# BDMstudio/audio-cut

Measured on AMD Instinct MI355X. Metric: audio-seconds processed/sec (separate+detect) per GPU; cut-point index parity, higher is better.
Workload: dtype f32

## Files before the change

### audio_cut_amd/_native.py

```python
from __future__ import annotations

import ctypes as C
import threading
import os
from pathlib import Path
from typing import Optional, Sequence, Tuple

import numpy as np
import torch

_LIB_NAME = "libaudiocut_hip.so"
_lib: Optional[C.CDLL] = None


class NativeError(RuntimeError):
    pass


def library_path() -> Path:
    return Path(__file__).resolve().parent / os.environ.get("AUDIOCUT_HIP_LIBNAME", _LIB_NAME)


def load() -> C.CDLL:
    global _lib
    if _lib is not None:
        return _lib
    path = library_path()
    if not path.exists():
        raise NativeError(f"{path} is missing: build it with `make -C audio_cut_amd/csrc` "
                          f"(there is no CPU fallback for the HIP path)")
    lib = C.CDLL(str(path))
    _declare(lib)
    if lib.ac_abi_version() != 6:
        raise NativeError("libaudiocut_hip.so ABI version mismatch")
    if lib.ac_stereo_abi_version() != 1:
        raise NativeError("libaudiocut_hip.so stereo ABI version mismatch")
    if lib.ac_onset_abi_version() != 1:
        raise NativeError("libaudiocut_hip.so onset ABI version mismatch")
    if lib.ac_beat_abi_version() != 1:
        raise NativeError("libaudiocut_hip.so beat ABI version mismatch")
    if lib.ac_hybrid_abi_version() != 1:
        raise NativeError("libaudiocut_hip.so hybrid ABI version mismatch")
    if lib.ac_export_abi_version() != 1:
        raise NativeError("libaudiocut_hip.so export ABI version mismatch")
    if lib.ac_asr_abi_version() != 1:
        raise NativeError("libaudiocut_hip.so asr ABI version mismatch")
    if lib.ac_profile_abi_version() != 1:
        raise NativeError("libaudiocut_hip.so profile ABI version mismatch")
    _lib = lib
    return lib


_P = C.c_void_p
_I64 = C.c_int64
_I = C.c_int

SIGNATURES = {
    "ac_abi_version": (C.c_int, []),
    "ac_last_error": (C.c_char_p, []),
    "ac_ctx_create": (C.c_int, [_I, C.POINTER(_P)]),
    "ac_ctx_destroy": (C.c_int, [_P]),
    "ac_frame_rms": (C.c_int, [_P, _P, _I64, _I, _I, _I, _P, _I64, _P]),
    "ac_frame_rms_multi": (C.c_int, [_P, _P, _I64, _I, _P, _P, _P, _P, _P]),
    "ac_stft2048_features": (C.c_int, [_P, _P, _I64, _I, _P, _P, _P, _P, _P, _I64, _P]),
    "ac_onset_strength": (C.c_int, [_P, _P, _I64, _P, _I, _I, _I, _P, _P, _P]),
    "ac_tempogram_parts": (C.c_int, [_I64]),
    "ac_tempogram_reduce": (C.c_int, [_P, _P, _I64, _I, _P, _P, _P, _P, _P]),
    "ac_yin_f0": (C.c_int, [_P, _P, _I64, _I, _I, _I, _I, C.c_double, _P, _P, _I64, _P]),
    "ac_moving_meansq_db_f64": (C.c_int, [_P, _P, _I64, _I, _P, _P]),
    "ac_next_leq_scratch": (C.c_int64, [_I64]),
    "ac_next_leq_scan": (C.c_int, [_P, _P, _I64, C.c_double, _P, _P, _P]),
    "ac_window_argmin_f64": (C.c_int, [_P, _P, _I64, _P, _P, _I, _P, _P, _P]),
    "ac_zero_cross_nearest": (C.c_int, [_P, _P, _I64, _P, _I, _I, _P, _P]),
    "ac_quiet_guard_slow": (C.c_int, [_P, _P, _I64, _P, _I, _I, _I, _P, _P, _P]),
    "ac_pause_cut_points": (C.c_int, [_P, _P, _I64, _P, _P, _I, _I, _I, _P, _P, _P]),
    "ac_mdx_stft": (C.c_int, [_P, _P, _I64, _P, _P, _P, _I, _P, _P, _P]),
    "ac_mdx_istft": (C.c_int, [_P, _P, _I, _P, _P, _P]),
    "ac_mdx_assemble_ola": (C.c_int, [_P, _P, _I64, _P, _P, _P, _P, _P, _P, _I, _P, _P, _P]),
    "ac_mdx_chunk_vocal": (C.c_int, [_P, _P, _P, _P, _P, _I, _P, _P]),
    "ac_sum_squares": (C.c_int, [_P, _P, _I64, _P, _I, _P]),
    "ac_window_sum_squares": (C.c_int, [_P, _P, _I64, _P, _P, _I, _P, _P]),
# ... 35 lines not shown


ONSET_SIGNATURES = {
    "ac_onset_abi_version": (C.c_int, []),
    "ac_bar_energy_silence": (C.c_int, [_P, _P, _I64, _P, _P, _I, C.c_double, _P, _P, _P]),
    "ac_segment_pair_energy": (C.c_int, [_P, _P, _P, _I64, _P, _P, _I, _P, _P]),
}

BEAT_SIGNATURES = {
    "ac_beat_abi_version": (C.c_int, []),
    "ac_stft2048_centroid_bandwidth": (C.c_int, [_P, _P, _I64, _I, C.c_double, _P, _P, _I64, _P]),
    "ac_bar_means3": (C.c_int, [_P, _P, _I64, _P, _P, _I64, _P, _P, _I, _P, _P]),
}

HYBRID_SIGNATURES = {
    "ac_hybrid_abi_version": (C.c_int, []),
    "ac_quiet_gate_meansq": (C.c_int, [_P, _P, _I64, _I64, _P, _I, _P, _I64, _P, _P, _P]),
}

EXPORT_SIGNATURES = {
    "ac_export_abi_version": (C.c_int, []),
    "ac_mdx_assemble_pcm24": (C.c_int, [_P, _P, _I64, _I, _P, _P, _P, _P, _P, _P, _I, _P, _P, _P, _I, _P]),
}

ASR_SIGNATURES = {
    "ac_asr_abi_version": (C.c_int, []),
    "ac_resample_poly_pcm16": (C.c_int, [_P, _P, _I64, _I, _I, _P, _I64, _I64, _P, _I64, _P]),
}

PROFILE_SIGNATURES = {
    "ac_profile_abi_version": (C.c_int, []),
    "ac_abs_peak_coverage": (C.c_int, [_P, _P, _I64, C.c_double, C.c_double, _P, _P, _P, _P]),
}
PROFILE_GRID_SAMPLES = 4 * 256 * 2048


def coverage_from(peak: float, count: int, n: int) -> float:
    if int(n) == 0 or float(peak) <= 1e-9:
        return 0.0
    return max(0.0, min(1.0, int(count) / int(n)))


def _declare(lib: C.CDLL) -> None:
    for name, (res, args) in (*SIGNATURES.items(), *STEREO_SIGNATURES.items(), *ONSET_SIGNATURES.items(), *BEAT_SIGNATURES.items(),
                              *HYBRID_SIGNATURES.items(), *EXPORT_SIGNATURES.items(), *ASR_SIGNATURES.items(), *PROFILE_SIGNATURES.items()):
        fn = getattr(lib, name)
        fn.restype = res
        fn.argtypes = args


def _check(rc: int) -> None:
    if rc != 0:
        msg = load().ac_last_error()
        raise NativeError(f"libaudiocut_hip call failed ({rc}): {msg.decode() if msg else '?'}")


def _ptr(t: Optional[torch.Tensor]) -> Optional[int]:
    if t is None:
        return None
    if not t.is_contiguous():
        raise NativeError("non-contiguous tensor passed to the HIP ABI")
    return t.data_ptr()


def _stream() -> int:
    return torch.cuda.current_stream().cuda_stream


def _packed(name: str, t: Optional[torch.Tensor], n_bytes: Optional[int]) -> None:
    if t is None or n_bytes is None:
        return
    have = t.numel() * t.element_size()
    if have != n_bytes:
        raise NativeError(f"{name}: the packed weights hold {have} bytes, the shape implies {n_bytes} (see separation/conv_pack.py)")


def _conv3x3_packed_bytes(c_in: int, c_out: int, cob: int, stage: int) -> Optional[int]:
    if c_in <= 0 or c_out <= 0 or c_in % 16 or c_out % cob:
# ... 708 lines not shown
    def conv3x3_f16x3_first(self, spec: torch.Tensor, w1: torch.Tensor, b1: torch.Tensor, w_packed: torch.Tensor, bias: torch.Tensor,
                            c_out: int, w_unscale: float, relu: bool = True, spec_amax: Optional[torch.Tensor] = None,
                            amax_gain: float = 1.0, amax_offs: float = 0.0, out_amax: Optional[torch.Tensor] = None) -> torch.Tensor:
        if spec.dtype != torch.float32 or spec.dim() != 4 or not spec.is_contiguous():
            raise NativeError("conv3x3_f16x3_first expects a contiguous float32 NCHW tensor")
        b, c0, h, w = spec.shape
        w1 = w1.reshape(w1.shape[0], -1)
        if w1.shape[1] != c0 or not w1.is_contiguous():
            raise NativeError("conv3x3_f16x3_first: w1 must be [C_in, C0(,1,1)] contiguous")
        _packed("conv3x3_f16x3_first", w_packed, _conv3x3_packed_bytes(w1.shape[0], int(c_out), 48, 8))
        out = torch.empty((b, c_out, h, w), dtype=torch.float32, device=self.device)
        pi, po = self._amax_args(b, spec_amax, out_amax, h, h)
        _check(self.lib.ac_conv3x3_f16x3_first(self._h, _ptr(spec), _ptr(w1), _ptr(b1), _ptr(w_packed), _ptr(bias), _ptr(out), b, c0,
                                               w1.shape[0], c_out, h, w, float(w_unscale), int(relu), pi, float(amax_gain),
                                               float(amax_offs), po, _stream()))
        return out

    def tdf_linear_f16x3(self, x: torch.Tensor, w_packed: torch.Tensor, n_out: int, scale: torch.Tensor, shift: torch.Tensor,
                         w_unscale: float, resid: Optional[torch.Tensor] = None, in_amax: Optional[torch.Tensor] = None,
                         out_amax: Optional[torch.Tensor] = None) -> torch.Tensor:
        if x.dtype != torch.float32 or x.dim() != 4 or not x.is_contiguous():
            raise NativeError("tdf_linear_f16x3 expects a contiguous float32 NCHW tensor")
        b, c, t, k = x.shape
        if c % 16 == 0 and t % 8 == 0:
            _packed("tdf_linear_f16x3", w_packed, _linear_packed_bytes(int(n_out), k, 0))
        out = torch.empty((b, c, t, n_out), dtype=torch.float32, device=self.device)
        if resid is not None and (resid.shape != out.shape or not resid.is_contiguous() or resid.dtype != torch.float32):
            raise NativeError("tdf_linear_f16x3: residual must match the output")
        pi, po = self._amax_args(b, in_amax, out_amax, t, t)
        _check(self.lib.ac_tdf_linear_f16x3(self._h, _ptr(x), _ptr(w_packed), _ptr(scale), _ptr(shift), _ptr(resid), _ptr(out),
                                            b * c * t, n_out, k, t, c, float(w_unscale), pi, po, _stream()))
        return out

    def tdf_small_fused(self, x: torch.Tensor, w1_packed: torch.Tensor, w2_packed: torch.Tensor, hidden: int, scale1: torch.Tensor,
                        shift1: torch.Tensor, scale2: torch.Tensor, shift2: torch.Tensor,
                        out_amax: Optional[torch.Tensor] = None) -> torch.Tensor:
        if x.dtype != torch.float32 or x.dim() != 4 or not x.is_contiguous():
            raise NativeError("tdf_small_fused expects a contiguous float32 NCHW tensor")
        b, c, t, f = x.shape
        hd = int(hidden)
        if f > 0 and f % 32 == 0 and 0 < hd <= 48 and (b * c * t) % 32 == 0:
            _packed("tdf_small_fused (w1)", w1_packed, -(-hd // 16) * (f // 16) * 64 * 4 * 4)
            _packed("tdf_small_fused (w2)", w2_packed, (f // 16) * -(-hd // 4) * 64 * 4)
        out = torch.empty_like(x)
        _, po = self._amax_args(b, None, out_amax, t, t)
        _check(self.lib.ac_tdf_small_fused(self._h, _ptr(x), _ptr(w1_packed), _ptr(w2_packed), _ptr(scale1), _ptr(shift1), _ptr(scale2),
                                           _ptr(shift2), _ptr(out), b * c * t, f, int(hidden), t, c, po, _stream()))
        return out

    def conv1x1_small(self, x: torch.Tensor, weight: torch.Tensor, bias: torch.Tensor, relu: bool) -> torch.Tensor:
        if x.dtype != torch.float32 or x.dim() != 4 or not x.is_contiguous():
            raise NativeError("conv1x1_small expects a contiguous float32 NCHW tensor")
        b, c, h, w = x.shape
        w2 = weight.reshape(weight.shape[0], -1)
        if w2.shape[1] != c or not w2.is_contiguous():
            raise NativeError("conv1x1_small: weight must be [C_out, C_in(,1,1)] contiguous")
        _packed("conv1x1_small (bias)", bias, w2.shape[0] * 4)
        out = torch.empty((b, w2.shape[0], h, w), dtype=torch.float32, device=self.device)
        _check(self.lib.ac_conv1x1_small(self._h, _ptr(x), _ptr(w2), _ptr(bias), _ptr(out), b, c, w2.shape[0], h * w, int(relu), _stream()))
        return out

    def down2x_f16x3(self, x: torch.Tensor, w_packed: torch.Tensor, bias: torch.Tensor, c_out: int, w_unscale: float,
                     in_amax: Optional[torch.Tensor] = None, out_amax: Optional[torch.Tensor] = None) -> torch.Tensor:
        if x.dtype != torch.float32 or x.dim() != 4 or not x.is_contiguous():
            raise NativeError("down2x_f16x3 expects a contiguous float32 NCHW tensor")
        b, c, h, w = x.shape
# ... 69 lines not shown
```

### audio_cut_amd/csrc/ac_gemm.hip

```cpp
#include "ac_common.h"
#include <stdlib.h>
#ifndef GM_RESID_AHEAD
#define GM_RESID_AHEAD 0
#endif
#ifndef AC_PROBES
#define AC_PROBES 0
#endif

typedef __attribute__((ext_vector_type(8))) _Float16 f16x8;
typedef __attribute__((ext_vector_type(4))) float f32x4;

#define GM_BM 128
#define GM_BK 32
#define GM_ASTRIDE 48
#define GM_MT 4
#define GM_A_ITERS ((GM_BM * (GM_BK / 4)) / 256)

__device__ inline unsigned short gm_f16_bits(_Float16 h) { return __builtin_bit_cast(unsigned short, h); }

template <int NT, bool RESID>
__global__ __launch_bounds__(256, 2) void k_tdf_linear_f16x3(const float* __restrict__ x, const f16x8* __restrict__ wpk,
                                                             const float* __restrict__ scale, const float* __restrict__ shift,
                                                             const float* __restrict__ resid, float* __restrict__ y,
                                                             int n_mblk, int N, int K, int T, int C, float w_unscale,
                                                             const float* __restrict__ in_amax, float* __restrict__ out_amax,
                                                             int ord_g, int ord_r) {
    constexpr int BN = 32 * NT;
    constexpr int BFRAGS = 2 * (BN / 16) * 64;
    constexpr int B_ITERS = BFRAGS / 256;
    constexpr int OSTRIDE = 16 * NT + 4;
    constexpr int A_BYTES = 2 * GM_BM * GM_ASTRIDE * 2;
    constexpr int O_BYTES = 4 * 16 * OSTRIDE * 4;
    constexpr int R_BYTES = (RESID && GM_RESID_AHEAD) ? 2 * (16 * (16 * NT) * 4) : 0;
    constexpr int K_ARENA = A_BYTES + 2 * BFRAGS * 16, E_ARENA = O_BYTES + 4 * R_BYTES;
    constexpr int ARENA = K_ARENA > E_ARENA ? K_ARENA : E_ARENA;
    __shared__ __attribute__((aligned(16))) unsigned char s_raw[ARENA];
    unsigned short* s_hi = reinterpret_cast<unsigned short*>(s_raw);
    unsigned short* s_lo = s_hi + GM_BM * GM_ASTRIDE;
    f16x8* s_b0 = reinterpret_cast<f16x8*>(s_raw + A_BYTES);
    f16x8* s_b1 = s_b0 + BFRAGS;
    float* s_out = reinterpret_cast<float*>(s_raw);

    const int tid = threadIdx.x, lane = tid & 63, wave = tid >> 6;
    const int wm = wave >> 1, wn = wave & 1;
    const int n_nblk = N / BN;
    int wi = blockIdx.x;
    if ((gridDim.x & 7) == 0) wi = (blockIdx.x & 7) * (gridDim.x >> 3) + (blockIdx.x >> 3);
    const int per = ord_r * n_nblk;
    const int chunk = wi / per, i_in = wi - chunk * per;
    const int nb_hi = i_in / (ord_g * ord_r), j_in = i_in - nb_hi * (ord_g * ord_r);
    const int nb = nb_hi * ord_g + j_in % ord_g, mb = chunk * ord_r + j_in / ord_g;
    if (mb >= n_mblk) return;
    const int n0 = nb * BN;
    const int n_stage = K / GM_BK;
    const int n_blk = T / 8, n_cg = C / 16;
    const int tb = mb % n_blk, cg = (mb / n_blk) % n_cg, item = mb / (n_blk * n_cg);
    const size_t m_base = ((size_t)item * C + (size_t)cg * 16) * T + (size_t)tb * 8;
    auto grow = [&](int r) -> size_t { return m_base + (size_t)(r >> 3) * T + (r & 7); };
    __shared__ float s_scale[8], s_inv[8];
    __shared__ unsigned s_tmax[8];
    if (tid < 8) {
        float inv;
        s_scale[tid] = ac_act_scale_lane(in_amax ? in_amax + (size_t)item * T : nullptr, tb * 8 + tid, tb * 8 + tid, &inv);
        s_inv[tid] = inv;
        s_tmax[tid] = 0u;
    }

    f32x4 acc[GM_MT][NT];
#pragma unroll
    for (int m = 0; m < GM_MT; ++m)
#pragma unroll
        for (int n = 0; n < NT; ++n) acc[m][n] = (f32x4){0.f, 0.f, 0.f, 0.f};

    const float* a_ptr[GM_A_ITERS];
    int a_off[GM_A_ITERS];
#pragma unroll
    for (int i = 0; i < GM_A_ITERS; ++i) {
        const int e = tid + 256 * i;
        const int row = e >> 3, kq = e & 7;
        a_ptr[i] = x + grow(row) * (size_t)K + 4 * kq;
        a_off[i] = row * GM_ASTRIDE + 4 * kq;
    }
    const f16x8* wbase = wpk + (size_t)nb * n_stage * BFRAGS;

    float4 pre_a[GM_A_ITERS];
    auto prefetch = [&](int s) {
        f16x8* dst = (s & 1) ? s_b1 : s_b0;
#pragma unroll
        for (int i = 0; i < B_ITERS; ++i) {
            const int inst = wave + 4 * i;
            __builtin_amdgcn_global_load_lds(wbase + (size_t)s * BFRAGS + inst * 64 + lane, dst + inst * 64, 16, 0, 0);
        }
#pragma unroll
        for (int i = 0; i < GM_A_ITERS; ++i) pre_a[i] = *reinterpret_cast<const float4*>(a_ptr[i] + (size_t)s * GM_BK);
    };
    prefetch(0);
    __syncthreads();
    float a_scale[GM_A_ITERS];
#pragma unroll
    for (int i = 0; i < GM_A_ITERS; ++i) a_scale[i] = s_scale[((tid + 256 * i) >> 3) & 7];

    const int frag_row = lane & 15, frag_k = 8 * (lane >> 4);
    for (int s = 0; s < n_stage; ++s) {
        __syncthreads();
        const f16x8* s_b = (s & 1) ? s_b1 : s_b0;
#pragma unroll
        for (int i = 0; i < GM_A_ITERS; ++i) {
            const float v[4] = {pre_a[i].x, pre_a[i].y, pre_a[i].z, pre_a[i].w};
            unsigned short h[4], l[4];
#pragma unroll
            for (int q = 0; q < 4; ++q) {
                const float c = fminf(fmaxf(v[q] * a_scale[i], -65504.f), 65504.f);
                const _Float16 hv = (_Float16)c;
                h[q] = gm_f16_bits(hv);
                l[q] = gm_f16_bits((_Float16)(c - (float)hv));
            }
            *reinterpret_cast<uint2*>(&s_hi[a_off[i]]) = make_uint2((unsigned)h[0] | ((unsigned)h[1] << 16), (unsigned)h[2] | ((unsigned)h[3] << 16));
            *reinterpret_cast<uint2*>(&s_lo[a_off[i]]) = make_uint2((unsigned)l[0] | ((unsigned)l[1] << 16), (unsigned)l[2] | ((unsigned)l[3] << 16));
        }
        __builtin_amdgcn_s_waitcnt(0);
        __syncthreads();
        if (s + 1 < n_stage) prefetch(s + 1);
        f16x8 ah[GM_MT], al[GM_MT];
#pragma unroll
        for (int m = 0; m < GM_MT; ++m) {
            const int off = (wm * 64 + m * 16 + frag_row) * GM_ASTRIDE + frag_k;
            ah[m] = *reinterpret_cast<const f16x8*>(&s_hi[off]);
            al[m] = *reinterpret_cast<const f16x8*>(&s_lo[off]);
        }
#pragma unroll
        for (int n = 0; n < NT; ++n) {
            const f16x8 bh = s_b[(0 * (BN / 16) + wn * NT + n) * 64 + lane];
            const f16x8 bl = s_b[(1 * (BN / 16) + wn * NT + n) * 64 + lane];
#pragma unroll
            for (int m = 0; m < GM_MT; ++m) {
                acc[m][n] = __builtin_amdgcn_mfma_f32_16x16x32_f16(ah[m], bl, acc[m][n], 0, 0, 0);
                acc[m][n] = __builtin_amdgcn_mfma_f32_16x16x32_f16(al[m], bh, acc[m][n], 0, 0, 0);
                acc[m][n] = __builtin_amdgcn_mfma_f32_16x16x32_f16(ah[m], bh, acc[m][n], 0, 0, 0);
            }
        }
    }
    const int g = lane >> 4, px = lane & 15;
    float* so = s_out + wave * 16 * OSTRIDE;
    constexpr int ROW_F4 = 4 * NT;
    constexpr int E_ITERS = 16 * ROW_F4 / 64;
    float4 rr[2][E_ITERS];
    auto out_offset = [&](int m, int i, int& c) -> size_t {
        const int e = lane + 64 * i;
        const int row = e / ROW_F4, q4 = e - row * ROW_F4;
        const int tr = wm * 64 + m * 16 + row;
        c = cg * 16 + (tr >> 3);
        return grow(tr) * (size_t)N + n0 + wn * (16 * NT) + 4 * q4;
    };
#if GM_RESID_AHEAD
    static_assert(GM_MT == 4, "the residual prefetch is laid out for four strips");
    unsigned char* s_res = s_raw + O_BYTES + wave * R_BYTES;
    if (RESID) {
#pragma unroll
        for (int m = 2; m < 4; ++m)
#pragma unroll
            for (int i = 0; i < E_ITERS; ++i) { int c; rr[m - 2][i] = *reinterpret_cast<const float4*>(resid + out_offset(m, i, c)); }
    }
    __syncthreads();
    if (RESID) {
#pragma unroll
        for (int m = 0; m < 2; ++m)
#pragma unroll
            for (int i = 0; i < E_ITERS; ++i) { int c; ac_lds_dma16(resid + out_offset(m, i, c), s_res + (m * E_ITERS + i) * 1024); }
    }
    float vm[E_ITERS];
#pragma unroll
    for (int i = 0; i < E_ITERS; ++i) vm[i] = 0.f;
#pragma unroll
    for (int m = 0; m < GM_MT; ++m) {
#pragma unroll
        for (int n = 0; n < NT; ++n)
#pragma unroll
            for (int r = 0; r < 4; ++r) so[(g * 4 + r) * OSTRIDE + n * 16 + px] = acc[m][n][r];
        if (RESID && m == 0) __builtin_amdgcn_s_waitcnt(0);
        __builtin_amdgcn_wave_barrier();
#pragma unroll
        for (int i = 0; i < E_ITERS; ++i) {
            const int e = lane + 64 * i;
            const int row = e / ROW_F4, q4 = e - row * ROW_F4;
            int c;
            const size_t o = out_offset(m, i, c);
            const int tr = wm * 64 + m * 16 + row;
            const float sc = scale[c] * (w_unscale * s_inv[tr & 7]), sh = shift[c];
            float4 v = *reinterpret_cast<const float4*>(&so[row * OSTRIDE + 4 * q4]);
            v.x = fmaxf(v.x * sc + sh, 0.f); v.y = fmaxf(v.y * sc + sh, 0.f);
            v.z = fmaxf(v.z * sc + sh, 0.f); v.w = fmaxf(v.w * sc + sh, 0.f);
            if (RESID) {
                const float4 q = m >= 2 ? rr[m - 2][i] : *reinterpret_cast<const float4*>(s_res + (m * E_ITERS + i) * 1024 + lane * 16);
                v.x += q.x; v.y += q.y; v.z += q.z; v.w += q.w;
            }
            vm[i] = fmaxf(fmaxf(vm[i], fmaxf(fabsf(v.x), fabsf(v.y))), fmaxf(fabsf(v.z), fabsf(v.w)));
            *reinterpret_cast<float4*>(y + o) = v;
        }
        __builtin_amdgcn_wave_barrier();
    }
#else
    if (RESID) {
#pragma unroll
        for (int i = 0; i < E_ITERS; ++i) { int c; rr[0][i] = *reinterpret_cast<const float4*>(resid + out_offset(0, i, c)); }
    }
    __syncthreads();
    float vm[E_ITERS];
#pragma unroll
    for (int i = 0; i < E_ITERS; ++i) vm[i] = 0.f;
#pragma unroll
    for (int m = 0; m < GM_MT; ++m) {
#pragma unroll
        for (int n = 0; n < NT; ++n)
#pragma unroll
            for (int r = 0; r < 4; ++r) so[(g * 4 + r) * OSTRIDE + n * 16 + px] = acc[m][n][r];
        if (RESID && m + 1 < GM_MT) {
#pragma unroll
            for (int i = 0; i < E_ITERS; ++i) { int c; rr[(m + 1) & 1][i] = *reinterpret_cast<const float4*>(resid + out_offset(m + 1, i, c)); }
        }
        __builtin_amdgcn_wave_barrier();
#pragma unroll
        for (int i = 0; i < E_ITERS; ++i) {
            const int e = lane + 64 * i;
            const int row = e / ROW_F4, q4 = e - row * ROW_F4;
            int c;
            const size_t o = out_offset(m, i, c);
            const int tr = wm * 64 + m * 16 + row;
            const float sc = scale[c] * (w_unscale * s_inv[tr & 7]), sh = shift[c];
            float4 v = *reinterpret_cast<const float4*>(&so[row * OSTRIDE + 4 * q4]);
            v.x = fmaxf(v.x * sc + sh, 0.f); v.y = fmaxf(v.y * sc + sh, 0.f);
            v.z = fmaxf(v.z * sc + sh, 0.f); v.w = fmaxf(v.w * sc + sh, 0.f);
            if (RESID) { const float4 q = rr[m & 1][i]; v.x += q.x; v.y += q.y; v.z += q.z; v.w += q.w; }
            vm[i] = fmaxf(fmaxf(vm[i], fmaxf(fabsf(v.x), fabsf(v.y))), fmaxf(fabsf(v.z), fabsf(v.w)));
            *reinterpret_cast<float4*>(y + o) = v;
        }
        __builtin_amdgcn_wave_barrier();
    }
#endif
    if (out_amax) {
#pragma unroll
        for (int i = 0; i < E_ITERS; ++i) {
            float a = fmaxf(vm[i], __shfl_xor(vm[i], 1, AC_WAVE));
            a = fmaxf(a, __shfl_xor(a, 2, AC_WAVE));
            if ((lane & 3) == 0) atomicMax(&s_tmax[((lane + 64 * i) / ROW_F4) & 7], __float_as_uint(a));
        }
        __syncthreads();
        if (tid < 8 && s_tmax[tid]) atomicMax(reinterpret_cast<unsigned*>(out_amax + (size_t)item * T + tb * 8 + tid), s_tmax[tid]);
    }
}

extern "C" int ac_tdf_linear_f16x3(ac_ctx* ctx, const float* x, const void* w_packed, const float* scale, const float* shift,
                                    const float* resid, float* y, long long M, int N, int K, int T, int C, float w_unscale,
                                    const float* in_amax, float* out_amax, void* stream) {
    AC_REQUIRE(ctx && x && w_packed && scale && shift && y, "null pointer");
    AC_REQUIRE(M > 0 && C > 0 && T > 0 && C % 16 == 0 && T % 8 == 0 && M % ((long long)C * T) == 0,
               "rows = items x C x T with C % 16 == 0 and T % 8 == 0 (a tile is 16 channels x 8 time rows)");
    AC_REQUIRE(K > 0 && K % GM_BK == 0, "K % 32 == 0");
    AC_REQUIRE(N > 0 && N % 96 == 0, "N % 96 == 0");
    const bool wide = (N % 192) == 0;
    const long long n_mblk = M / GM_BM;
    const int n_nblk = N / (wide ? 192 : 96);
    long long nblk = n_mblk * n_nblk;
    AC_REQUIRE(nblk < (1LL << 31) - 8 && n_mblk < (1LL << 31), "grid too large");
    int ord_g = n_nblk, ord_r = 1;
    if (n_nblk % 4 == 0 && n_nblk > 4 && n_mblk % 16 == 0) { ord_g = 4; ord_r = 16; }
#if AC_PROBES
    if (const char* e = getenv("AC_PROBE_TDF_ORDER")) {
        int g_ = 0, r_ = 0;
        if (sscanf(e, "%d,%d", &g_, &r_) == 2 && g_ > 0 && r_ > 0 && n_nblk % g_ == 0 && n_mblk % r_ == 0) { ord_g = g_; ord_r = r_; }
    }
#endif
    dim3 grid((unsigned)nblk), block(256);
    hipStream_t st = (hipStream_t)stream;
    const f16x8* wp = (const f16x8*)w_packed;
#define GM_GO(NT_, RES_) hipLaunchKernelGGL((k_tdf_linear_f16x3<NT_, RES_>), grid, block, 0, st, x, wp, scale, shift, resid, y, (int)n_mblk, N, K, T, C, w_unscale, in_amax, out_amax, ord_g, ord_r)
    if (wide) { if (resid) GM_GO(6, true); else GM_GO(6, false); }
    else      { if (resid) GM_GO(3, true); else GM_GO(3, false); }
#undef GM_GO
    AC_LAUNCH_CHECK();
    return AC_OK;
}
```

### audio_cut_amd/separation/tfc_tdf.py

```python
from __future__ import annotations

from dataclasses import dataclass
from typing import Dict, List, Optional

import numpy as np
import torch
import torch.nn as nn

Weights = Dict[str, np.ndarray]


@dataclass(frozen=True)
class TfcTdfSpec:
    dim_c: int = 4
    dim_f: int = 3072
    dim_t: int = 256
    n_levels: int = 5
    l: int = 3
    g: int = 48
    k: int = 3
    bn: int = 8
    bn_eps: float = 1e-5

    def channels(self, level: int) -> int:
# ... 102 lines not shown
        self._w_unscale = []
        for j in range(self.l):
            w = getattr(self, f"cw{j}").detach().cpu().numpy()
            if w.shape[0] % 48 or w.shape[1] % 16:
                self._w_unscale.append(None)
                continue
            if conv3x3_wide_tileable(w.shape[0], w.shape[1]):
                wide, unscale = pack_conv3x3_w96(w, 96)
                self.register_buffer(f"cwq{j}", torch.from_numpy(wide.view(np.int16)).to(dev))
            else:
                narrow, unscale = pack_conv3x3_w96(w, 48)
                self.register_buffer(f"cws{j}", torch.from_numpy(narrow.view(np.int16)).to(dev))
            self._w_unscale.append(unscale)

    def _conv(self, x: torch.Tensor, ax: torch.Tensor, j: int, hip, tape: _AmaxTape, probe):
        from .._native import NativeError
        if x.shape[2] % 8 or x.shape[3] % 32 or not (hasattr(self, f"cwq{j}") or hasattr(self, f"cws{j}")):
            raise NativeError(f"3x3 conv of shape {tuple(x.shape)} is not tileable by the HIP kernels (C % 48, C_in % 16, H % 8, W % 32)")
        if probe is not None:
            e0 = torch.cuda.Event(enable_timing=True); e1 = torch.cuda.Event(enable_timing=True)
            e0.record()
        ay = tape.new(x.shape[2])
        if hasattr(self, f"cwq{j}"):
            y = hip.conv3x3_f16x3_w96(x, getattr(self, f"cwq{j}"), getattr(self, f"cb{j}"), x.shape[1], self._w_unscale[j], relu=True,
                                      in_amax=ax, out_amax=ay)
        else:
            y = hip.conv3x3_f16x3_s8(x, getattr(self, f"cws{j}"), getattr(self, f"cb{j}"), x.shape[1], self._w_unscale[j], relu=True,
                                     in_amax=ax, out_amax=ay)
        if probe is not None:
            e1.record()
            probe.append((e0, e1, 2.0 * x.shape[0] * x.shape[1] * x.shape[1] * 9 * x.shape[2] * x.shape[3]))
        return y, ay

    def _tdf(self, x: torch.Tensor, ax: torch.Tensor, hip, tape: _AmaxTape):
        from .._native import NativeError
        rows = x.shape[0] * x.shape[1] * x.shape[2]
        ay = tape.new(x.shape[2])
        if hasattr(self, "lwp0") and x.shape[1] % 16 == 0 and x.shape[2] % 8 == 0:
            ah = tape.new(x.shape[2])
            h = hip.tdf_linear_f16x3(x, self.lwp0, self.lw0.shape[0], self.ls0.view(-1), self.lb0.view(-1), self._l_unscale[0],
                                     in_amax=ax, out_amax=ah)
            y = hip.tdf_linear_f16x3(h, self.lwp1, self.lw1.shape[0], self.ls1.view(-1), self.lb1.view(-1), self._l_unscale[1], resid=x,
                                     in_amax=ah, out_amax=ay)
            return y, ay
        if hasattr(self, "lws0") and rows % 32 == 0 and (x.shape[1] * x.shape[2]) % 32 == 0:
            y = hip.tdf_small_fused(x, self.lws0, self.lws1, self.lw0.shape[0], self.ls0.view(-1), self.lb0.view(-1),
                                    self.ls1.view(-1), self.lb1.view(-1), out_amax=ay)
            return y, ay
        raise NativeError(f"TDF of shape {tuple(x.shape)} -> {self.lw0.shape[0]} is not tileable by the HIP kernels")

    def forward_hip(self, x: torch.Tensor, ax: torch.Tensor, hip, tape: _AmaxTape, probe=None, first=None):
        start = 0
        if first is not None:
            if probe is not None:
                e0 = torch.cuda.Event(enable_timing=True); e1 = torch.cuda.Event(enable_timing=True)
                e0.record()
            spec = x
            ay = tape.new(x.shape[2])
            if not hasattr(self, "cws0"):
                from .._native import NativeError
                raise NativeError("the fused first conv needs a 48-output-channel-tileable 3x3 conv behind the 1x1 (ac_conv3x3_f16x3_first)")
            x = hip.conv3x3_f16x3_first(spec, first[0], first[1], self.cws0, self.cb0, self.cw0.shape[0], self._w_unscale[0], relu=True,
                                        spec_amax=ax, amax_gain=first[2], amax_offs=first[3], out_amax=ay)
            ax = ay
            if probe is not None:
                e1.record()
                c = self.cw0.shape[0]
                probe.append((e0, e1, 2.0 * spec.shape[0] * c * c * 9 * spec.shape[2] * spec.shape[3]))
            start = 1
        for j in range(start, self.l):
            x, ax = self._conv(x, ax, j, hip, tape, probe)
        return self._tdf(x, ax, hip, tape)


class TfcTdfNet(nn.Module):

    def __init__(self, weights: Weights, spec: TfcTdfSpec = TfcTdfSpec(), hip=None):
        super().__init__()
        self.spec = spec
        self.hip = hip
        self.conv_probe = None
        self.block_tap = None
        w = weights
        wf, bf = _fold(w["first_conv.weight"], w["first_conv.bias"], w, "first_bn", spec.bn_eps, 0)
        self.register_buffer("first_w", torch.from_numpy(wf))
        self.register_buffer("first_b", torch.from_numpy(bf))
        self._first_gain = float(np.max(np.sum(np.abs(wf.reshape(wf.shape[0], -1).astype(np.float64)), axis=1)))
        self._first_offs = float(np.max(np.abs(bf.astype(np.float64)))) if bf.size else 0.0
        self.enc = nn.ModuleList(_Block(w, f"enc.{i}", spec) for i in range(spec.n_levels))
        self.dec = nn.ModuleList(_Block(w, f"dec.{i}", spec) for i in range(spec.n_levels))
        self.bottleneck = _Block(w, "bottleneck", spec)
        for i in range(spec.n_levels):
            wf, bf = _fold(w[f"ds.{i}.conv.weight"], w[f"ds.{i}.conv.bias"], w, f"ds.{i}.bn", spec.bn_eps, 0)
            self.register_buffer(f"ds_w{i}", torch.from_numpy(wf))
            self.register_buffer(f"ds_b{i}", torch.from_numpy(bf))
            wf, bf = _fold(w[f"us.{i}.conv.weight"], w[f"us.{i}.conv.bias"], w, f"us.{i}.bn", spec.bn_eps, 1)
            self.register_buffer(f"us_w{i}", torch.from_numpy(wf))
            self.register_buffer(f"us_b{i}", torch.from_numpy(bf))
        if hip is not None:
            from .conv_pack import pack_linear
            for blk in [*self.enc, *self.dec, self.bottleneck]:
                blk.pack_for_hip()
            self._rs_unscale = {}
            for i in range(spec.n_levels):
                dsw = getattr(self, f"ds_w{i}").numpy()
# ... 28 lines not shown
                           in_amax=ax, out_amax=ay)
        return y, ay

    @torch.no_grad()
    def forward(self, spec_in: torch.Tensor) -> torch.Tensor:
        return self.forward_tf(spec_in.transpose(-1, -2).contiguous()).transpose(-1, -2)

    @torch.no_grad()
    def forward_tf(self, spec_tf: torch.Tensor, spec_amax: Optional[torch.Tensor] = None) -> torch.Tensor:
        from .._native import NativeError
        hip = self.hip
        if hip is None or not spec_tf.is_cuda:
            raise NativeError("TfcTdfNet runs on the HIP kernels only: construct it with hip=Context and feed device tensors "
                              "(tests/unet_torch.py holds the PyTorch reference evaluation)")
        n = self.spec.n_levels
        b, c0, t, f = spec_tf.shape
        if not spec_tf.is_contiguous() or c0 > 4 or self.first_w.shape[0] > 64 or t % 8 or f % 32 or not hasattr(self.enc[0], "cws0"):
            raise NativeError(f"spectrogram of shape {tuple(spec_tf.shape)} is not tileable by ac_conv3x3_f16x3_first")
        if spec_amax is None:
            spec_amax = spec_tf.abs().amax(dim=(1, 3)).view(b, t // AMAX_ROWS, AMAX_ROWS).amax(dim=2).contiguous()
        tape = _AmaxTape(b, t, 6 * (2 * n + 1) + 2 * n, spec_tf.device)
        skips = []
        x, ax = spec_tf, spec_amax
        for i in range(n):
            first = (self.first_w, self.first_b, self._first_gain, self._first_offs) if i == 0 else None
            x, ax = self.enc[i].forward_hip(x, ax, hip, tape, self.conv_probe, first=first)
            if self.block_tap is not None: self.block_tap(f"enc{i}", x)
            skips.append(x)
            x, ax = self._down(x, ax, i, hip, tape)
        x, ax = self.bottleneck.forward_hip(x, ax, hip, tape, self.conv_probe)
        if self.block_tap is not None: self.block_tap("bottleneck", x)
        for i in range(n):
            x, ax = self._up(x, ax, i, hip, skips.pop(), tape)
            x, ax = self.dec[i].forward_hip(x, ax, hip, tape, self.conv_probe)
            if self.block_tap is not None: self.block_tap(f"dec{i}", x)
        return hip.conv1x1_small(x, self.final_w, self.final_b, relu=False)
```

Before: 1543.

## Fuse final 1x1 conv into last decoder TDF linear epilogue

Adds a FINAL variant of the f16x3 TDF linear kernel that tiles 48 channels x 2 time rows, so one tile holds every channel of its pixels. The epilogue applies scale/shift/ReLU and the residual, then runs the final 1x1 conv to C_out in shared memory and writes the output spectrogram directly. This avoids writing the full 48-channel decoder output and reading it back in a separate conv1x1_small launch. The trade-off is a smaller M tile (96 vs 128), which may lower MFMA efficiency, plus extra epilogue work and shared memory.

After: 1560, median of 6. 1.1% higher.

```diff
diff --git a/audio_cut_amd/_native.py b/audio_cut_amd/_native.py
--- a/audio_cut_amd/_native.py
+++ b/audio_cut_amd/_native.py
@@ -47,6 +47,8 @@
         raise NativeError("libaudiocut_hip.so asr ABI version mismatch")
     if lib.ac_profile_abi_version() != 1:
         raise NativeError("libaudiocut_hip.so profile ABI version mismatch")
+    if lib.ac_final_abi_version() != 1:
+        raise NativeError("libaudiocut_hip.so final-layer ABI version mismatch")
     _lib = lib
     return lib
 
@@ -148,6 +150,10 @@
     "ac_profile_abi_version": (C.c_int, []),
     "ac_abs_peak_coverage": (C.c_int, [_P, _P, _I64, C.c_double, C.c_double, _P, _P, _P, _P]),
 }
+FINAL_SIGNATURES = {
+    "ac_final_abi_version": (C.c_int, []),
+    "ac_tdf_linear_final_f16x3": (C.c_int, [_P, _P, _P, _P, _P, _P, _P, _P, _P, _P, _I64, _I, _I, _I, _I, _I, C.c_float, _P, _P]),
+}
 PROFILE_GRID_SAMPLES = 4 * 256 * 2048
 
 
@@ -159,7 +165,8 @@
 
 def _declare(lib: C.CDLL) -> None:
     for name, (res, args) in (*SIGNATURES.items(), *STEREO_SIGNATURES.items(), *ONSET_SIGNATURES.items(), *BEAT_SIGNATURES.items(),
-                              *HYBRID_SIGNATURES.items(), *EXPORT_SIGNATURES.items(), *ASR_SIGNATURES.items(), *PROFILE_SIGNATURES.items()):
+                              *HYBRID_SIGNATURES.items(), *EXPORT_SIGNATURES.items(), *ASR_SIGNATURES.items(), *PROFILE_SIGNATURES.items(),
+                              *FINAL_SIGNATURES.items()):
         fn = getattr(lib, name)
         fn.restype = res
         fn.argtypes = args
@@ -934,6 +941,35 @@
                                             b * c * t, n_out, k, t, c, float(w_unscale), pi, po, _stream()))
         return out
 
+    @staticmethod
+    def tdf_final_tileable(c: int, t: int, k: int, n_out: int, c_out: int) -> bool:
+        return c == 48 and t > 0 and t % 2 == 0 and k > 0 and k % 32 == 0 and n_out > 0 and n_out % 192 == 0 and 1 <= c_out <= 4
+
+    def tdf_linear_final_f16x3(self, x: torch.Tensor, w_packed: torch.Tensor, n_out: int, scale: torch.Tensor, shift: torch.Tensor,
+                               w_unscale: float, resid: torch.Tensor, final_w: torch.Tensor, final_b: torch.Tensor,
+                               in_amax: Optional[torch.Tensor] = None, want_y: bool = False):
+        if x.dtype != torch.float32 or x.dim() != 4 or not x.is_contiguous():
+            raise NativeError("tdf_linear_final_f16x3 expects a contiguous float32 NCHW tensor")
+        b, c, t, k = x.shape
+        w2 = final_w.reshape(final_w.shape[0], -1)
+        if w2.shape[1] != c or not w2.is_contiguous() or w2.dtype != torch.float32:
+            raise NativeError("tdf_linear_final_f16x3: final weight must be [C_out, C(,1,1)] contiguous float32")
+        c_out = w2.shape[0]
+        if self.tdf_final_tileable(c, t, k, int(n_out), c_out):
+            _packed("tdf_linear_final_f16x3", w_packed, _linear_packed_bytes(int(n_out), k, 0))
+        _packed("tdf_linear_final_f16x3 (bias)", final_b, c_out * 4)
+        _packed("tdf_linear_final_f16x3 (scale)", scale, c * 4)
+        _packed("tdf_linear_final_f16x3 (shift)", shift, c * 4)
+        if resid is None or resid.shape != (b, c, t, n_out) or not resid.is_contiguous() or resid.dtype != torch.float32:
+            raise NativeError("tdf_linear_final_f16x3: residual must match the TDF layer's output")
+        spec = torch.empty((b, c_out, t, n_out), dtype=torch.float32, device=self.device)
+        y = torch.empty((b, c, t, n_out), dtype=torch.float32, device=self.device) if want_y else None
+        pi, _ = self._amax_args(b, in_amax, None, t, t)
+        _check(self.lib.ac_tdf_linear_final_f16x3(self._h, _ptr(x), _ptr(w_packed), _ptr(scale), _ptr(shift), _ptr(resid), _ptr(w2),
+                                                  _ptr(final_b), _ptr(spec), _ptr(y), b * c * t, n_out, k, t, c, c_out,
+                                                  float(w_unscale), pi, _stream()))
+        return (spec, y) if want_y else spec
+
     def tdf_small_fused(self, x: torch.Tensor, w1_packed: torch.Tensor, w2_packed: torch.Tensor, hidden: int, scale1: torch.Tensor,
                         shift1: torch.Tensor, scale2: torch.Tensor, shift2: torch.Tensor,
                         out_amax: Optional[torch.Tensor] = None) -> torch.Tensor:
diff --git a/audio_cut_amd/csrc/ac_gemm.hip b/audio_cut_amd/csrc/ac_gemm.hip
--- a/audio_cut_amd/csrc/ac_gemm.hip
+++ b/audio_cut_amd/csrc/ac_gemm.hip
@@ -1,4 +1,5 @@
 #include "ac_common.h"
+#include "../../include/audiocut_hip_final.h"
 #include <stdlib.h>
 #ifndef GM_RESID_AHEAD
 #define GM_RESID_AHEAD 0
@@ -11,32 +12,38 @@
 typedef __attribute__((ext_vector_type(4))) float f32x4;
 
 #define GM_BM 128
+#define GM_BM_FINAL 96
 #define GM_BK 32
 #define GM_ASTRIDE 48
-#define GM_MT 4
-#define GM_A_ITERS ((GM_BM * (GM_BK / 4)) / 256)
 
 __device__ inline unsigned short gm_f16_bits(_Float16 h) { return __builtin_bit_cast(unsigned short, h); }
 
-template <int NT, bool RESID>
+template <int NT, bool RESID, int BM = GM_BM, int TR = 8, bool FINAL = false>
 __global__ __launch_bounds__(256, 2) void k_tdf_linear_f16x3(const float* __restrict__ x, const f16x8* __restrict__ wpk,
                                                              const float* __restrict__ scale, const float* __restrict__ shift,
                                                              const float* __restrict__ resid, float* __restrict__ y,
                                                              int n_mblk, int N, int K, int T, int C, float w_unscale,
                                                              const float* __restrict__ in_amax, float* __restrict__ out_amax,
-                                                             int ord_g, int ord_r) {
+                                                             int ord_g, int ord_r, const float* __restrict__ fin_w = nullptr,
+                                                             const float* __restrict__ fin_b = nullptr, float* __restrict__ spec = nullptr,
+                                                             int C_out = 0) {
+    static_assert(FINAL ? (BM == 96 && NT == 6 && RESID) : (BM == 128 && TR == 8), "row tiles: 16 channels x 8 time rows, or 48 x 2 with the final 1x1 conv");
+    constexpr int MT = BM / 32;
+    constexpr int A_ITERS = (BM * (GM_BK / 4)) / 256;
+    constexpr int CH = BM / TR;
     constexpr int BN = 32 * NT;
     constexpr int BFRAGS = 2 * (BN / 16) * 64;
     constexpr int B_ITERS = BFRAGS / 256;
     constexpr int OSTRIDE = 16 * NT + 4;
-    constexpr int A_BYTES = 2 * GM_BM * GM_ASTRIDE * 2;
+    constexpr int A_BYTES = 2 * BM * GM_ASTRIDE * 2;
     constexpr int O_BYTES = 4 * 16 * OSTRIDE * 4;
     constexpr int R_BYTES = (RESID && GM_RESID_AHEAD) ? 2 * (16 * (16 * NT) * 4) : 0;
-    constexpr int K_ARENA = A_BYTES + 2 * BFRAGS * 16, E_ARENA = O_BYTES + 4 * R_BYTES;
+    constexpr int TSTRIDE = BN + 4;
+    constexpr int K_ARENA = A_BYTES + 2 * BFRAGS * 16, E_ARENA = FINAL ? BM * TSTRIDE * 4 : O_BYTES + 4 * R_BYTES;
     constexpr int ARENA = K_ARENA > E_ARENA ? K_ARENA : E_ARENA;
     __shared__ __attribute__((aligned(16))) unsigned char s_raw[ARENA];
     unsigned short* s_hi = reinterpret_cast<unsigned short*>(s_raw);
-    unsigned short* s_lo = s_hi + GM_BM * GM_ASTRIDE;
+    unsigned short* s_lo = s_hi + BM * GM_ASTRIDE;
     f16x8* s_b0 = reinterpret_cast<f16x8*>(s_raw + A_BYTES);
     f16x8* s_b1 = s_b0 + BFRAGS;
     float* s_out = reinterpret_cast<float*>(s_raw);
@@ -53,29 +60,29 @@
     if (mb >= n_mblk) return;
     const int n0 = nb * BN;
     const int n_stage = K / GM_BK;
-    const int n_blk = T / 8, n_cg = C / 16;
+    const int n_blk = T / TR, n_cg = C / CH;
     const int tb = mb % n_blk, cg = (mb / n_blk) % n_cg, item = mb / (n_blk * n_cg);
-    const size_t m_base = ((size_t)item * C + (size_t)cg * 16) * T + (size_t)tb * 8;
-    auto grow = [&](int r) -> size_t { return m_base + (size_t)(r >> 3) * T + (r & 7); };
-    __shared__ float s_scale[8], s_inv[8];
-    __shared__ unsigned s_tmax[8];
-    if (tid < 8) {
+    const size_t m_base = ((size_t)item * C + (size_t)cg * CH) * T + (size_t)tb * TR;
+    auto grow = [&](int r) -> size_t { return m_base + (size_t)(r / TR) * T + (r % TR); };
+    __shared__ float s_scale[TR], s_inv[TR];
+    __shared__ unsigned s_tmax[TR];
+    if (tid < TR) {
         float inv;
-        s_scale[tid] = ac_act_scale_lane(in_amax ? in_amax + (size_t)item * T : nullptr, tb * 8 + tid, tb * 8 + tid, &inv);
+        s_scale[tid] = ac_act_scale_lane(in_amax ? in_amax + (size_t)item * T : nullptr, tb * TR + tid, tb * TR + tid, &inv);
         s_inv[tid] = inv;
         s_tmax[tid] = 0u;
     }
 
-    f32x4 acc[GM_MT][NT];
-#pragma unroll
-    for (int m = 0; m < GM_MT; ++m)
+    f32x4 acc[MT][NT];
+#pragma unroll
+    for (int m = 0; m < MT; ++m)
 #pragma unroll
         for (int n = 0; n < NT; ++n) acc[m][n] = (f32x4){0.f, 0.f, 0.f, 0.f};
 
-    const float* a_ptr[GM_A_ITERS];
-    int a_off[GM_A_ITERS];
-#pragma unroll
-    for (int i = 0; i < GM_A_ITERS; ++i) {
+    const float* a_ptr[A_ITERS];
+    int a_off[A_ITERS];
+#pragma unroll
+    for (int i = 0; i < A_ITERS; ++i) {
         const int e = tid + 256 * i;
         const int row = e >> 3, kq = e & 7;
         a_ptr[i] = x + grow(row) * (size_t)K + 4 * kq;
@@ -83,7 +90,7 @@
     }
     const f16x8* wbase = wpk + (size_t)nb * n_stage * BFRAGS;
 
-    float4 pre_a[GM_A_ITERS];
+    float4 pre_a[A_ITERS];
     auto prefetch = [&](int s) {
         f16x8* dst = (s & 1) ? s_b1 : s_b0;
 #pragma unroll
@@ -92,20 +99,20 @@
             __builtin_amdgcn_global_load_lds(wbase + (size_t)s * BFRAGS + inst * 64 + lane, dst + inst * 64, 16, 0, 0);
         }
 #pragma unroll
-        for (int i = 0; i < GM_A_ITERS; ++i) pre_a[i] = *reinterpret_cast<const float4*>(a_ptr[i] + (size_t)s * GM_BK);
+        for (int i = 0; i < A_ITERS; ++i) pre_a[i] = *reinterpret_cast<const float4*>(a_ptr[i] + (size_t)s * GM_BK);
     };
     prefetch(0);
     __syncthreads();
-    float a_scale[GM_A_ITERS];
-#pragma unroll
-    for (int i = 0; i < GM_A_ITERS; ++i) a_scale[i] = s_scale[((tid + 256 * i) >> 3) & 7];
+    float a_scale[A_ITERS];
+#pragma unroll
+    for (int i = 0; i < A_ITERS; ++i) a_scale[i] = s_scale[((tid + 256 * i) >> 3) % TR];
 
     const int frag_row = lane & 15, frag_k = 8 * (lane >> 4);
     for (int s = 0; s < n_stage; ++s) {
         __syncthreads();
         const f16x8* s_b = (s & 1) ? s_b1 : s_b0;
 #pragma unroll
-        for (int i = 0; i < GM_A_ITERS; ++i) {
+        for (int i = 0; i < A_ITERS; ++i) {
             const float v[4] = {pre_a[i].x, pre_a[i].y, pre_a[i].z, pre_a[i].w};
             unsigned short h[4], l[4];
 #pragma unroll
@@ -121,10 +128,10 @@
         __builtin_amdgcn_s_waitcnt(0);
         __syncthreads();
         if (s + 1 < n_stage) prefetch(s + 1);
-        f16x8 ah[GM_MT], al[GM_MT];
-#pragma unroll
-        for (int m = 0; m < GM_MT; ++m) {
-            const int off = (wm * 64 + m * 16 + frag_row) * GM_ASTRIDE + frag_k;
+        f16x8 ah[MT], al[MT];
+#pragma unroll
+        for (int m = 0; m < MT; ++m) {
+            const int off = (wm * (BM / 2) + m * 16 + frag_row) * GM_ASTRIDE + frag_k;
             ah[m] = *reinterpret_cast<const f16x8*>(&s_hi[off]);
             al[m] = *reinterpret_cast<const f16x8*>(&s_lo[off]);
         }
@@ -133,12 +140,88 @@
             const f16x8 bh = s_b[(0 * (BN / 16) + wn * NT + n) * 64 + lane];
             const f16x8 bl = s_b[(1 * (BN / 16) + wn * NT + n) * 64 + lane];
 #pragma unroll
-            for (int m = 0; m < GM_MT; ++m) {
+            for (int m = 0; m < MT; ++m) {
                 acc[m][n] = __builtin_amdgcn_mfma_f32_16x16x32_f16(ah[m], bl, acc[m][n], 0, 0, 0);
                 acc[m][n] = __builtin_amdgcn_mfma_f32_16x16x32_f16(al[m], bh, acc[m][n], 0, 0, 0);
                 acc[m][n] = __builtin_amdgcn_mfma_f32_16x16x32_f16(ah[m], bh, acc[m][n], 0, 0, 0);
             }
         }
+    }
+    if constexpr (FINAL) {
+        constexpr int WR = BM / 2, WC = BN / 2;
+        constexpr int ROW_F4 = WC / 4;
+        constexpr int P_ITERS = 16 * ROW_F4 / 64;
+        const int g = lane >> 4, px = lane & 15;
+        float* s_tile = reinterpret_cast<float*>(s_raw);
+        float* sw = s_tile + wm * WR * TSTRIDE + wn * WC;
+        auto y_offset = [&](int m, int i, int& tr) -> size_t {
+            const int e = lane + 64 * i;
+            const int row = e / ROW_F4, q4 = e - row * ROW_F4;
+            tr = wm * WR + m * 16 + row;
+            return grow(tr) * (size_t)N + n0 + wn * WC + 4 * q4;
+        };
+        float4 rr[2][P_ITERS];
+#pragma unroll
+        for (int i = 0; i < P_ITERS; ++i) { int tr; rr[0][i] = *reinterpret_cast<const float4*>(resid + y_offset(0, i, tr)); }
+        __syncthreads();
+#pragma unroll
+        for (int m = 0; m < MT; ++m)
+#pragma unroll
+            for (int n = 0; n < NT; ++n)
+#pragma unroll
+                for (int r = 0; r < 4; ++r) sw[(m * 16 + g * 4 + r) * TSTRIDE + n * 16 + px] = acc[m][n][r];
+        __builtin_amdgcn_wave_barrier();
+#pragma unroll
+        for (int m = 0; m < MT; ++m) {
+            if (m + 1 < MT) {
+#pragma unroll
+                for (int i = 0; i < P_ITERS; ++i) { int tr; rr[(m + 1) & 1][i] = *reinterpret_cast<const float4*>(resid + y_offset(m + 1, i, tr)); }
+            }
+#pragma unroll
+            for (int i = 0; i < P_ITERS; ++i) {
+                const int e = lane + 64 * i;
+                const int row = e / ROW_F4, q4 = e - row * ROW_F4;
+                int tr;
+                const size_t o = y_offset(m, i, tr);
+                const int c = cg * CH + tr / TR;
+                const float sc = scale[c] * (w_unscale * s_inv[tr % TR]), sh = shift[c];
+                float4* cell = reinterpret_cast<float4*>(&sw[(m * 16 + row) * TSTRIDE + 4 * q4]);
+                float4 v = *cell;
+                v.x = fmaxf(v.x * sc + sh, 0.f); v.y = fmaxf(v.y * sc + sh, 0.f);
+                v.z = fmaxf(v.z * sc + sh, 0.f); v.w = fmaxf(v.w * sc + sh, 0.f);
+                const float4 q = rr[m & 1][i];
+                v.x += q.x; v.y += q.y; v.z += q.z; v.w += q.w;
+                *cell = v;
+                if (y) *reinterpret_cast<float4*>(y + o) = v;
+            }
+        }
+        __syncthreads();
+        if (tid < TR * (BN / 2)) {
+            const int t = tid / (BN / 2), cp = tid - t * (BN / 2);
+            const float* tp = s_tile + t * TSTRIDE + 2 * cp;
+            int cw[4];
+            float2 a[4];
+#pragma unroll
+            for (int co = 0; co < 4; ++co) {
+                cw[co] = co < C_out ? co : 0;
+                const float bv = fin_b[cw[co]];
+                a[co] = make_float2(bv, bv);
+            }
+#pragma unroll
+            for (int c = 0; c < CH; ++c) {
+                const float2 v = *reinterpret_cast<const float2*>(tp + c * TR * TSTRIDE);
+#pragma unroll
+                for (int co = 0; co < 4; ++co) {
+                    const float wv = fin_w[cw[co] * CH + c];
+                    a[co].x = fmaf(wv, v.x, a[co].x); a[co].y = fmaf(wv, v.y, a[co].y);
+                }
+            }
+#pragma unroll
+            for (int co = 0; co < 4; ++co)
+                if (co < C_out)
+                    *reinterpret_cast<float2*>(spec + (((size_t)item * C_out + co) * T + (size_t)tb * TR + t) * N + n0 + 2 * cp) = a[co];
+        }
+        return;
     }
     const int g = lane >> 4, px = lane & 15;
     float* so = s_out + wave * 16 * OSTRIDE;
@@ -153,7 +236,7 @@
         return grow(tr) * (size_t)N + n0 + wn * (16 * NT) + 4 * q4;
     };
 #if GM_RESID_AHEAD
-    static_assert(GM_MT == 4, "the residual prefetch is laid out for four strips");
+    static_assert(MT == 4, "the residual prefetch is laid out for four strips");
     unsigned char* s_res = s_raw + O_BYTES + wave * R_BYTES;
     if (RESID) {
 #pragma unroll
@@ -172,7 +255,7 @@
 #pragma unroll
     for (int i = 0; i < E_ITERS; ++i) vm[i] = 0.f;
 #pragma unroll
-    for (int m = 0; m < GM_MT; ++m) {
+    for (int m = 0; m < MT; ++m) {
 #pragma unroll
         for (int n = 0; n < NT; ++n)
 #pragma unroll
@@ -209,12 +292,12 @@
 #pragma unroll
     for (int i = 0; i < E_ITERS; ++i) vm[i] = 0.f;
 #pragma unroll
-    for (int m = 0; m < GM_MT; ++m) {
+    for (int m = 0; m < MT; ++m) {
 #pragma unroll
         for (int n = 0; n < NT; ++n)
 #pragma unroll
             for (int r = 0; r < 4; ++r) so[(g * 4 + r) * OSTRIDE + n * 16 + px] = acc[m][n][r];
-        if (RESID && m + 1 < GM_MT) {
+        if (RESID && m + 1 < MT) {
 #pragma unroll
             for (int i = 0; i < E_ITERS; ++i) { int c; rr[(m + 1) & 1][i] = *reinterpret_cast<const float4*>(resid + out_offset(m + 1, i, c)); }
         }
@@ -280,3 +363,33 @@
     AC_LAUNCH_CHECK();
     return AC_OK;
 }
+
+extern "C" int ac_final_abi_version(void) { return AC_FINAL_ABI_VERSION; }
+
+extern "C" int ac_tdf_linear_final_f16x3(ac_ctx* ctx, const float* x, const void* w_packed, const float* scale, const float* shift,
+                                          const float* resid, const float* final_w, const float* final_b, float* spec, float* y,
+                                          long long M, int N, int K, int T, int C, int C_out, float w_unscale, const float* in_amax,
+                                          void* stream) {
+    AC_REQUIRE(ctx && x && w_packed && scale && shift && spec, "null pointer");
+    AC_REQUIRE(resid, "the residual is required (this is the block's second TDF layer)");
+    AC_REQUIRE(final_w && final_b, "null pointer (final conv)");
+    AC_REQUIRE(C > 0 && GM_BM_FINAL % C == 0, "96 % C == 0 (a tile holds every channel of its pixels)");
+    AC_REQUIRE(C == 48, "C == 48 (the tile built is 48 channels x 2 time rows)");
+    AC_REQUIRE(T > 0 && T % (GM_BM_FINAL / C) == 0, "T % (96 / C) == 0");
+    AC_REQUIRE(M > 0 && M % ((long long)C * T) == 0, "rows = items x C x T");
+    AC_REQUIRE(N > 0 && N % 192 == 0, "N % 192 == 0");
+    AC_REQUIRE(K > 0 && K % GM_BK == 0, "K % 32 == 0");
+    AC_REQUIRE(C_out >= 1 && C_out <= 4, "1 <= C_out <= 4");
+    const long long n_mblk = M / GM_BM_FINAL;
+    const int n_nblk = N / 192;
+    const long long nblk = n_mblk * n_nblk;
+    AC_REQUIRE(nblk < (1LL << 31) - 8 && n_mblk < (1LL << 31), "grid too large");
+    int ord_g = n_nblk, ord_r = 1;
+    if (n_nblk % 4 == 0 && n_nblk > 4 && n_mblk % 16 == 0) { ord_g = 4; ord_r = 16; }
+    dim3 grid((unsigned)nblk), block(256);
+    hipLaunchKernelGGL((k_tdf_linear_f16x3<6, true, GM_BM_FINAL, 2, true>), grid, block, 0, (hipStream_t)stream, x, (const f16x8*)w_packed,
+                       scale, shift, resid, y, (int)n_mblk, N, K, T, C, w_unscale, in_amax, (float*)nullptr, ord_g, ord_r, final_w, final_b,
+                       spec, C_out);
+    AC_LAUNCH_CHECK();
+    return AC_OK;
+}
diff --git a/audio_cut_amd/separation/tfc_tdf.py b/audio_cut_amd/separation/tfc_tdf.py
--- a/audio_cut_amd/separation/tfc_tdf.py
+++ b/audio_cut_amd/separation/tfc_tdf.py
@@ -158,7 +158,12 @@
             probe.append((e0, e1, 2.0 * x.shape[0] * x.shape[1] * x.shape[1] * 9 * x.shape[2] * x.shape[3]))
         return y, ay
 
-    def _tdf(self, x: torch.Tensor, ax: torch.Tensor, hip, tape: _AmaxTape):
+    def takes_final(self, c: int, t: int, final_w: torch.Tensor) -> bool:
+        from .._native import Context
+        return (hasattr(self, "lwp0") and c % 16 == 0 and t % 8 == 0 and final_w.shape[1] == c
+                and Context.tdf_final_tileable(c, t, self.lw1.shape[1], self.lw1.shape[0], final_w.shape[0]))
+
+    def _tdf(self, x: torch.Tensor, ax: torch.Tensor, hip, tape: _AmaxTape, final=None):
         from .._native import NativeError
         rows = x.shape[0] * x.shape[1] * x.shape[2]
         ay = tape.new(x.shape[2])
@@ -166,6 +171,9 @@
             ah = tape.new(x.shape[2])
             h = hip.tdf_linear_f16x3(x, self.lwp0, self.lw0.shape[0], self.ls0.view(-1), self.lb0.view(-1), self._l_unscale[0],
                                      in_amax=ax, out_amax=ah)
+            if final is not None:
+                return hip.tdf_linear_final_f16x3(h, self.lwp1, self.lw1.shape[0], self.ls1.view(-1), self.lb1.view(-1),
+                                                  self._l_unscale[1], x, final[0], final[1], in_amax=ah), None
             y = hip.tdf_linear_f16x3(h, self.lwp1, self.lw1.shape[0], self.ls1.view(-1), self.lb1.view(-1), self._l_unscale[1], resid=x,
                                      in_amax=ah, out_amax=ay)
             return y, ay
@@ -175,7 +183,7 @@
             return y, ay
         raise NativeError(f"TDF of shape {tuple(x.shape)} -> {self.lw0.shape[0]} is not tileable by the HIP kernels")
 
-    def forward_hip(self, x: torch.Tensor, ax: torch.Tensor, hip, tape: _AmaxTape, probe=None, first=None):
+    def forward_hip(self, x: torch.Tensor, ax: torch.Tensor, hip, tape: _AmaxTape, probe=None, first=None, final=None):
         start = 0
         if first is not None:
             if probe is not None:
@@ -196,7 +204,7 @@
             start = 1
         for j in range(start, self.l):
             x, ax = self._conv(x, ax, j, hip, tape, probe)
-        return self._tdf(x, ax, hip, tape)
+        return self._tdf(x, ax, hip, tape, final)
 
 
 class TfcTdfNet(nn.Module):
@@ -291,6 +299,11 @@
         if self.block_tap is not None: self.block_tap("bottleneck", x)
         for i in range(n):
             x, ax = self._up(x, ax, i, hip, skips.pop(), tape)
-            x, ax = self.dec[i].forward_hip(x, ax, hip, tape, self.conv_probe)
+            final = None
+            if i == n - 1 and self.block_tap is None and self.dec[i].takes_final(x.shape[1], x.shape[2], self.final_w):
+                final = (self.final_w, self.final_b)
+            x, ax = self.dec[i].forward_hip(x, ax, hip, tape, self.conv_probe, final=final)
+            if final is not None:
+                return x
             if self.block_tap is not None: self.block_tap(f"dec{i}", x)
         return hip.conv1x1_small(x, self.final_w, self.final_b, relu=False)
diff --git a/include/audiocut_hip_final.h b/include/audiocut_hip_final.h
--- /dev/null
+++ b/include/audiocut_hip_final.h
@@ -0,0 +1,23 @@
+#ifndef AUDIOCUT_HIP_FINAL_H
+#define AUDIOCUT_HIP_FINAL_H
+
+#include "audiocut_hip.h"
+
+#ifdef __cplusplus
+extern "C" {
+#endif
+
+#define AC_FINAL_ABI_VERSION 1
+
+int ac_final_abi_version(void);
+
+int ac_tdf_linear_final_f16x3(ac_ctx* ctx, const float* x, const void* w_packed, const float* scale, const float* shift,
+                              const float* resid, const float* final_w, const float* final_b, float* spec, float* y,
+                              long long M, int N, int K, int T, int C, int C_out, float w_unscale, const float* in_amax,
+                              void* stream);
+
+#ifdef __cplusplus
+}
+#endif
+
+#endif
```
